# YukunXia/SuperPoint-Stereo-Visual-Odometry

Measured on AMD Instinct MI355X. Metric: stereo frames/sec (1241x376 KITTI), higher is better.
Workload: dtype f32

## Files before the change

### superpoint-stereo-visual-odometry_amd/csrc/conv_first_pre.hip.h

```cpp
#pragma once
#include <hip/hip_runtime.h>
#include <stdint.h>
#include "conv_mfma.hip.h"
#include "post.hip.h"

namespace spvo {

struct FirstPreArgs {
  const uint8_t *src[4];
  uint8_t *out_u8[4];
  size_t stride;
  int row_off, col_off, crop_rows, crop_cols, identity;
  ResizeTab tab;
  float *in_plane;
  size_t in_per_image;
  float *out;
  const float *w, *bias;
  int H, W, hp, wp, out_ctot, out_coff, cout;
};

template <bool RELU>
__global__ __launch_bounds__(256) void conv_first4_pre_kernel(const FirstPreArgs a) {
  constexpr int TW = 256, LW = TW + 4;
  __shared__ __attribute__((aligned(16))) float s[6 * LW];
  const int tid = threadIdx.x, img = blockIdx.z;
  const int x0 = blockIdx.x * TW, y0 = blockIdx.y * 4;
  const uint8_t *src = a.src[img];
  uint8_t *o8 = a.out_u8[img];
  float *ipl = a.in_plane + (size_t)img * a.in_per_image;
  auto stage = [&](const int cx, const int ry0, const int nrows) {
    const int gx = x0 - 1 + cx;
    const bool col_ok = gx >= 0 && gx < a.W;
    const int gxc = col_ok ? gx : 0;
    int xs0 = 0, xs1 = 0, a0 = 0, a1 = 0;
    if (!a.identity) { xs0 = a.tab.xi[gxc]; xs1 = min(xs0 + 1, a.crop_cols - 1); a0 = a.tab.xa0[gxc]; a1 = a.tab.xa1[gxc]; }
    int vv[6];
#pragma unroll
    for (int k = 0; k < 6; ++k) {
      if (k >= nrows) break;
      const int gy = y0 - 1 + ry0 + k;
      const int gyc = min(max(gy, 0), a.H - 1);
      if (a.identity) {
        vv[k] = src[(size_t)(a.row_off + gyc) * a.stride + a.col_off + gxc];
      } else {
        const int ys0 = a.tab.yi[gyc], ys1 = min(ys0 + 1, a.crop_rows - 1);
        const int b0 = a.tab.yb0[gyc], b1 = a.tab.yb1[gyc];
        const uint8_t *r0 = src + (size_t)(a.row_off + ys0) * a.stride + a.col_off;
        const uint8_t *r1 = src + (size_t)(a.row_off + ys1) * a.stride + a.col_off;
        const int h0 = (int)r0[xs0] * a0 + (int)r0[xs1] * a1;
        const int h1 = (int)r1[xs0] * a0 + (int)r1[xs1] * a1;
        const int v = (((b0 * (h0 >> 4)) >> 16) + ((b1 * (h1 >> 4)) >> 16) + 2) >> 2;
        vv[k] = min(max(v, 0), 255);
      }
    }
#pragma unroll
    for (int k = 0; k < 6; ++k) {
      if (k >= nrows) break;
      const int ry = ry0 + k, gy = y0 - 1 + ry;
      const bool ok = col_ok && gy >= 0 && gy < a.H;
      const float f = ok ? mul_rn((float)vv[k], 1.0f / 255.0f) : 0.f;
      if (ok && ry >= 1 && ry <= 4 && cx >= 1 && cx <= TW) {
        if (o8) o8[(size_t)gy * a.W + gx] = (uint8_t)vv[k];
        ipl[(size_t)(gy + PADY) * a.wp + (gx + PADX)] = f;
      }
      s[ry * LW + 3 + cx] = f;
    }
  };
  stage(tid, 0, 6);
  if (tid < 12) stage(TW + (tid & 1), tid >> 1, 1);
  __syncthreads();
  const int l = tid & 63, r = tid >> 6;
  const int x = x0 + 4 * l, y = y0 + r;
  if (x >= a.W || y >= a.H) return;
  float v[3][6];
#pragma unroll
  for (int ky = 0; ky < 3; ++ky) {
    const float *rp = s + (r + ky) * LW + 4 + 4 * l;
    const float4 m = *reinterpret_cast<const float4 *>(rp);
    v[ky][0] = rp[-1]; v[ky][1] = m.x; v[ky][2] = m.y; v[ky][3] = m.z; v[ky][4] = m.w; v[ky][5] = rp[4];
  }
  const size_t plane = (size_t)a.hp * a.wp;
  float *op = a.out + ((size_t)img * a.out_ctot + a.out_coff) * plane + (size_t)(y + PADY) * a.wp + (x + PADX);
  for (int co = 0; co < a.cout; ++co) {
    float sum[4];
#pragma unroll
    for (int i = 0; i < 4; ++i) {
      sum[i] = a.bias[co];
#pragma unroll
      for (int t = 0; t < 9; ++t) sum[i] = fmaf(a.w[co * 9 + t], v[t / 3][i + t % 3], sum[i]);
      if (RELU) sum[i] = fmaxf(sum[i], 0.f);
    }
    *reinterpret_cast<float4 *>(op + (size_t)co * plane) = make_float4(sum[0], sum[1], sum[2], sum[3]);
  }
}

}
```

### superpoint-stereo-visual-odometry_amd/csrc/spvo_core.hip

```cpp
#include "spvo_internal.hip.h"
#include <mutex>

namespace spvo_int {

thread_local std::string g_error;
HostDiag g_diag;

int fail(spvo_ctx *c, int code, const char *fmt, ...) {
  char buf[512];
  va_list ap;
  va_start(ap, fmt);
  vsnprintf(buf, sizeof buf, fmt, ap);
  va_end(ap);
  if (c) c->error = buf;
  g_error = buf;
  return code;
}

int stage_id(spvo_ctx *c, const std::string &name) {
  for (size_t i = 0; i < c->stages.size(); ++i)
    if (c->stages[i].name == name) return (int)i;
  Stage s;
  s.name = name;
  c->stages.push_back(s);
  return (int)c->stages.size() - 1;
}

namespace {
const char *const kTuningNames[] = {"winograd", "wino4", "wino4_item", "wino_narrow", "wino_dynamic", "winograd_min_tiles", "wino4_min_tiles", "merge_siblings", "heads_fused",
                                    "heads_on_net", "heads_split", "match_fused", "fp32_split", "prematch", "spin_wait", "trunk_timing", "solve_timing", "nms_first", "upload_side", "inject_launch_failure", "int8_fused", "pair_always", "preprocess_fused", "heads_keep_raw", "tail_streams", "solve_collect_first", "graphs", "solve_fuse", "solve_keep", "sift_describe_form", "sift_pair_waves_per_cu", "sift_brisk_recheck", "conv_variant"};
constexpr int kTuningCount = sizeof kTuningNames / sizeof kTuningNames[0];
std::mutex g_tuning_mutex;
bool g_tuning_set[kTuningCount] = {};
int g_tuning_value[kTuningCount] = {};
int tuning_index(const char *name) {
  for (int i = 0; name && i < kTuningCount; ++i)
    if (std::strcmp(name, kTuningNames[i]) == 0) return i;
  return -1;
}
}
int tuning(const char *name, int dflt) {
  const int i = tuning_index(name);
  if (i < 0) return dflt;
  std::lock_guard<std::mutex> lock(g_tuning_mutex);
  return g_tuning_set[i] ? g_tuning_value[i] : dflt;
}

bool spin_wait_enabled() { return tuning("spin_wait", 0) != 0; }
hipError_t wait_event(hipEvent_t ev) {
  if (spin_wait_enabled()) {
    for (long spins = 0; spins < 20000000; ++spins) {
      const hipError_t e = hipEventQuery(ev);
      if (e != hipErrorNotReady) return e;
      __builtin_ia32_pause();
    }
  }
  return hipEventSynchronize(ev);
}

hipEvent_t get_event(spvo_ctx *c) {
  if (!c->free_events.empty()) {
    hipEvent_t e = c->free_events.back();
    c->free_events.pop_back();
    return e;
  }
  hipEvent_t e;
  (void)hipEventCreate(&e);
  return e;
}

void resolve_pending(spvo_ctx *c) {
  if (c->pending.empty()) return;
  for (auto &p : c->pending) {
    float ms = 0;
    (void)hipEventSynchronize(p.e1);
    if (hipEventElapsedTime(&ms, p.e0, p.e1) == hipSuccess) {
      c->stages[p.stage].total_ms += ms;
      c->stages[p.stage].calls += 1;
      c->stages[p.stage].flops_sum += p.flops;
      c->stages[p.stage].bytes_sum += p.bytes;
    }
    c->free_events.push_back(p.e0);
    c->free_events.push_back(p.e1);
  }
  c->pending.clear();
}

__thread LaunchRecorder *t_rec = nullptr;

static void seg_drop(GraphEntry &e) {
  if (e.exec) (void)hipGraphExecDestroy(e.exec);
  if (e.graph) (void)hipGraphDestroy(e.graph);
  e = GraphEntry();
}

void set_release_segments(SubmitSet &s) {
  for (GraphEntry *e : {&s.seg_T[0], &s.seg_T[1], &s.seg_H[0], &s.seg_H[1], &s.seg_A, &s.seg_B}) seg_drop(*e);
}
void seg_free_all(spvo_ctx *c) {
  for (SubmitSet &s : c->sets) set_release_segments(s);
}

void seg_abort(spvo_ctx *c) {
  LaunchRecorder &r = c->rec;
  if (t_rec == &r) t_rec = nullptr;
  r.active = false; r.poisoned = false;
  r.rec.clear();
}

bool seg_begin(spvo_ctx *c, GraphEntry *e, hipStream_t stream) {
  LaunchRecorder &r = c->rec;
  if (t_rec == &r) seg_abort(c);
  if (!c->use_graphs || !e || e->never || t_rec) return false;
// ... 412 lines not shown
```

### superpoint-stereo-visual-odometry_amd/csrc/spvo_detect.hip

```cpp
#include "spvo_internal.hip.h"
#include "conv_mfma.hip.h"
#include "post.hip.h"
#include "conv_first_pre.hip.h"

namespace spvo_int {

static void linear_coeffs(int dst, int src, std::vector<int> &idx, std::vector<int> &a0, std::vector<int> &a1) {
  const double scale = (double)src / (double)dst;
  idx.resize(dst); a0.resize(dst); a1.resize(dst);
  for (int d = 0; d < dst; ++d) {
    float f = (float)((d + 0.5) * scale - 0.5);
    int s = (int)std::floor(f);
    f -= (float)s;
    if (s < 0) { s = 0; f = 0.f; }
    if (s >= src - 1) { s = src - 1; f = 0.f; }
    idx[d] = s;
    a0[d] = (int)std::nearbyint((1.f - f) * 2048.f);
    a1[d] = (int)std::nearbyint(f * 2048.f);
  }
}

void resize_tables(int dst_w, int src_w, int dst_h, int src_h, std::vector<int> &out) {
  std::vector<int> xi, xa0, xa1, yi, yb0, yb1;
  linear_coeffs(dst_w, src_w, xi, xa0, xa1);
// ... 14 lines not shown
  }
  g.scale = (float)net_w / (float)g.crop_cols;
  return g;
}

void fix_projection(double P[12], const CropGeom &g, int rows, int cols, int bug_compat) {
  if (bug_compat) {
    float lo;
    if (g.crop_rows != rows) {
      std::memcpy(&lo, (char *)&P[4 + 1], 4);
      lo -= (float)g.row_off;
      std::memcpy((char *)&P[4 + 1], &lo, 4);
    } else if (g.crop_cols != cols) {
      std::memcpy(&lo, (char *)&P[0 + 1], 4);
      lo -= (float)g.col_off;
      std::memcpy((char *)&P[0 + 1], &lo, 4);
    }
  } else {
    if (g.crop_rows != rows) P[4 + 2] -= (double)(float)g.row_off;
    else if (g.crop_cols != cols) P[0 + 2] -= (double)(float)g.col_off;
  }
  for (int k = 0; k < 8; ++k) P[k] *= (double)g.scale;
}

int ensure_tables(spvo_ctx *c, const CropGeom &g) {
  if (c->tab_rows == g.crop_rows && c->tab_cols == g.crop_cols) return SPVO_OK;
  std::vector<int> all;
  resize_tables(c->W, g.crop_cols, c->H, g.crop_rows, all);
  HIP_TRY(c, hipMemcpyAsync(c->d_tab, all.data(), all.size() * sizeof(int), hipMemcpyHostToDevice, c->stream));
  HIP_TRY(c, hipStreamSynchronize(c->stream));
  c->tab_rows = g.crop_rows;
  c->tab_cols = g.crop_cols;
  return SPVO_OK;
}

static ResizeTab resize_tab(const spvo_ctx *c) {
  ResizeTab t;
  t.xi = c->d_tab; t.xa0 = c->d_tab + c->W; t.xa1 = c->d_tab + 2 * c->W;
  t.yi = c->d_tab + 3 * c->W; t.yb0 = t.yi + c->H; t.yb1 = t.yi + 2 * c->H;
  return t;
}

static int ensure_img_staging(spvo_ctx *c, size_t bytes) {
  if (bytes <= c->d_img[1].count()) return SPVO_OK;
  return grow(c, wait_for_nothing(), {plain(c->d_img[0], bytes), plain(c->d_img[1], bytes)});
}

int launch_preprocess(spvo_ctx *c, const uint8_t *d_src0, const uint8_t *d_src1, int count, int rows, int cols, size_t stride, const CropGeom &g, int slot0,
                      uint8_t *resized_dst = nullptr) {
  int rc = ensure_tables(c, g);
  if (rc) return rc;
  ResizeTab tab = resize_tab(c);
  const Tensor &tin = c->tensors[c->t_input];
  const int identity = (g.crop_rows == c->H && g.crop_cols == c->W) ? 1 : 0;
  dim3 grid((c->W + 63) / 64, (c->H + 3) / 4, count);
  hipLaunchKernelGGL(preprocess_kernel, grid, dim3(256), 0, c->stream, d_src0, d_src1, stride, rows, cols, g.row_off, g.col_off, g.crop_rows, g.crop_cols, tab, c->H, c->W,
                     resized_dst ? resized_dst : c->d_resized + (size_t)(slot0 & 1) * c->H * c->W, tin.d + (size_t)slot0 * tin.per_image, tin.per_image, tin.hp, tin.wp, identity);
  HIP_TRY(c, hipGetLastError());
  return SPVO_OK;
}

int launch_first_pre(spvo_ctx *c, PendingDetect *const *mem, int n, hipStream_t stream) {
  const Op &op = c->ops[0];
  const Tensor &ti = c->tensors[op.in], &to = c->tensors[op.out];
  const CropGeom &g = mem[0]->g;
  FirstPreArgs a;
  for (int k = 0; k < 4; ++k) { a.src[k] = nullptr; a.out_u8[k] = nullptr; }
  const size_t hw = (size_t)c->H * c->W;
  for (int m = 0; m < n; ++m)
    for (int i = 0; i < 2; ++i) {
      a.src[2 * m + i] = mem[m]->src[i];
      a.out_u8[2 * m + i] = mem[m]->res_dst ? mem[m]->res_dst + i * hw : (m == n - 1 ? c->d_resized + i * hw : nullptr);
    }
  a.stride = mem[0]->stride;
  a.row_off = g.row_off; a.col_off = g.col_off; a.crop_rows = g.crop_rows; a.crop_cols = g.crop_cols;
  a.identity = (g.crop_rows == c->H && g.crop_cols == c->W) ? 1 : 0;
  a.tab = resize_tab(c);
  a.in_plane = ti.d; a.in_per_image = ti.per_image;
  a.out = ring_ptr(c, to);
  a.w = op.d_w; a.bias = op.d_b;
  a.H = ti.H; a.W = ti.W; a.hp = ti.hp; a.wp = ti.wp; a.out_ctot = to.ch; a.out_coff = op.out_c_off; a.cout = op.cout;
  const int batch = 2 * n;
  ScopedStage st(c, op.stage, op.flops_per_image * batch, 0.0, stream);
  const dim3 grid((ti.W + 255) / 256, (ti.H + 3) / 4, batch);
  if (op.flags & FLAG_RELU) hipLaunchKernelGGL(conv_first4_pre_kernel<true>, grid, dim3(256), 0, stream, a);
  else hipLaunchKernelGGL(conv_first4_pre_kernel<false>, grid, dim3(256), 0, stream, a);
  HIP_TRY(c, hipGetLastError());
  return SPVO_OK;
}

constexpr int NMS_INNER = 4;
constexpr int NMS_GRID = 128;

NmsPair nms_pair(const SubmitSet &s, int *counters) {
  NmsPair p;
  for (int i = 0; i < 2; ++i) {
    p.b[i] = s.nms[i];
    p.b[i].counters = counters + (size_t)i * NMS_COUNTER_INTS;
  }
  return p;
}

int launch_nms_rounds(spvo_ctx *c, int nimg, const NmsPair &np, const SubmitSet &s, int n_launch, int *zero_next, bool redo = false) {
  hipStream_t st = c->post;
  const float *heat = s.d_heat;
  const int collect = redo ? 0 : 1;
  const int n_round = (!redo && n_launch > 1) ? n_launch - 1 : n_launch;
  for (int l = 0; l < n_round; ++l) {
    if (c->cfg.dist_thresh == 4)
      hipLaunchKernelGGL((nms_round_kernel<NMS_INNER, 4>), dim3(NMS_GRID, nimg), dim3(256), 0, st, heat, c->H, c->W, 4, np, l, c->cfg.border_remove, c->surv_cap, collect);
    else
      hipLaunchKernelGGL((nms_round_kernel<NMS_INNER, 0>), dim3(NMS_GRID, nimg), dim3(256), 0, st, heat, c->H, c->W, c->cfg.dist_thresh, np, l, c->cfg.border_remove, c->surv_cap, collect);
  }
  if (n_round < n_launch) {
    if (c->cfg.dist_thresh == 4)
      hipLaunchKernelGGL((nms_finish_kernel<4>), dim3(nimg), dim3(NMS_FIN_THREADS), 0, st, heat, c->H, c->W, 4, np, n_round, c->cfg.border_remove, c->surv_cap);
    else
      hipLaunchKernelGGL((nms_finish_kernel<0>), dim3(nimg), dim3(NMS_FIN_THREADS), 0, st, heat, c->H, c->W, c->cfg.dist_thresh, np, n_round, c->cfg.border_remove, c->surv_cap);
  }
  if (redo) hipLaunchKernelGGL(nms_collect_kernel, dim3(NMS_GRID, nimg), dim3(256), 0, st, heat, c->H, c->W, c->cfg.border_remove, c->surv_cap, np);
  hipLaunchKernelGGL(nms_rank_kernel, dim3(128, nimg), dim3(256), 0, st, c->surv_cap, np);
  hipLaunchKernelGGL(nms_write_kernel, dim3(32, nimg), dim3(256), 0, st, c->H, c->cfg.max_keypoints, c->surv_cap, np, zero_next, s.h_counters);
  HIP_TRY(c, hipGetLastError());
  return SPVO_OK;
}


int nms_settle(spvo_ctx *c, int nimg, const NmsPair &np, const SubmitSet &s, bool *redone) {
  int last = c->nms_first;
  *redone = false;
  const int *hc = s.h_counters;
  for (;;) {
    bool pending = false;
    for (int i = 0; i < nimg; ++i) pending |= hc[i * NMS_COUNTER_INTS + 8 + last - 1] != 0;
    if (!pending) break;
    if (!*redone) c->stages[stage_id(c, "nms_redo")].calls += 1;
    *redone = true;
    last = NMS_MAX_LAUNCH;
    for (int i = 0; i < nimg; ++i)
      HIP_TRY(c, hipMemsetAsync(np.b[i].counters + 1, 0, (NMS_COUNTER_INTS - 1) * sizeof(int), c->post));
    int rc = launch_nms_rounds(c, nimg, np, s, last, nullptr, true);
    if (rc) return rc;
    HIP_TRY(c, hipStreamSynchronize(c->post));
  }
  for (int i = 0; i < nimg; ++i)
    if (hc[i * NMS_COUNTER_INTS + 3]) return fail(c, SPVO_ERR_CAPACITY, "NMS survivor buffer overflow");
  return SPVO_OK;
}

int run_nms(spvo_ctx *c, int nimg) {
  SubmitSet &s = standalone(c);
  const NmsPair np = nms_pair(s, c->d_counters_alone);
  for (int i = 0; i < nimg; ++i) HIP_TRY(c, hipMemsetAsync(np.b[i].counters, 0, NMS_COUNTER_INTS * sizeof(int), c->stream));
  dim3 grid((c->W + 63) / 64, (c->H + 3) / 4, nimg);
  hipLaunchKernelGGL(nms_threshold_kernel, grid, dim3(256), 0, c->stream, s.d_heat, c->H, c->W, c->cfg.conf_thresh, np);
  int rc = launch_nms_rounds(c, nimg, np, s, c->nms_first, nullptr);
  if (rc) return rc;
  HIP_TRY(c, hipStreamSynchronize(c->stream));
  bool redone;
  return nms_settle(c, nimg, np, s, &redone);
}

}

extern "C" {

int spvo_preprocess(spvo_ctx *c, const uint8_t *img, int rows, int cols, size_t stride, double P[12], uint8_t *resized_u8) {
  if (!c || !img || !P || rows <= 0 || cols <= 0 || stride < (size_t)cols) return fail(c, SPVO_ERR_INVALID, "bad argument");
  if (int rc = require_idle(c)) return rc;
// ... 588 lines not shown
```

### superpoint-stereo-visual-odometry_amd/csrc/spvo_internal.hip.h

```cpp
#pragma once
#include <hip/hip_runtime.h>

#include <algorithm>
#include <cmath>
#include <cstdarg>
#include <cstdio>
#include <cstdlib>
#include <cstring>
#include <string>
#include <vector>
#include <deque>
#include <functional>
#include <time.h>

#include "../../include/spvo.h"
#include "spvo_types.hip.h"
#include "engine_file.h"

#pragma GCC visibility push(hidden)
#include "dev_buf.h"
namespace spvo { struct BriskLongPair; struct BriskShortPair; }
using namespace spvo;

#include "launch_segments.hip.h"
// ... 408 lines not shown
    DevBuf<AkazeKp> sup_kp;
    int brk_cap = 0;
    DevBuf<BriskDetKeypoint> brk_rec, brk_crec;
    DevBuf<int> brk_keep, brk_cnt;
  } akaze;
  struct SiftBufs {
    int rows = 0, cols = 0;
    SiftPyr plan{};
    bool gauss_only = false;
    int first = -1;
    DevBuf<SiftKey> given_kp;
    DevBuf<float> given_desc;
    int given_cap = 0;
    int cand_cap = 0;
    DevBuf<uint8_t> img;
    DevBuf<float> pyr, desc;
    DevBuf<int4> cand_pos;
    DevBuf<float4> cand_off;
    DevBuf<int2> kp;
    DevBuf<int> counters;
    std::vector<int4> h_pos;
    std::vector<float4> h_off;
    std::vector<int2> h_kp;
    std::vector<float> h_desc;
    std::vector<spvo_sift_keypoint> h_rec;
    std::vector<int> h_order;
    int ord_cap = 0;
    DevBuf<SiftKey> keys;
    DevBuf<int> sorted, order;
    DevBuf<int> ord_n;
    int slot_cap = 0;
    SiftSlot slots[N_SIFT_SLOTS];
    PairStage pair;
    PinBuf<SiftSrc> h_src;
    PinBuf<float> hm_desc;
    PinBuf<int> h_n;
    PinBuf<int2> h_match;
    int h_match_cap = 0;
    bool match_pending = false;
    int lnk_cap = 0;
    DevBuf<int> lnk_kept, lnk_cnt, lnk_keep;
    int brk_cap = 0;
    DevBuf<BriskDetKeypoint> brk_rec, brk_crec;
    DevBuf<int> brk_keep, brk_cnt;
    PinBuf<SiftSrc> hb_src;
    PinBuf<int> hb_n;
    std::vector<BriskDetKeypoint> hb_rec;
  } sift;
  int ham_cap = 0;
  DevBuf<uint32_t> d_ham_a, d_ham_b;
  DevBuf<int> d_ham_idx;
  DevBuf<float> d_ham_dist;
  DevBuf<unsigned long long> d_ham_vote;
  DevBuf<int2> d_ham_out;
  int bin_pm_norm = SPVO_NORM_HAMMING;
  static constexpr int SOLVE_SLOTS = 3;
  static constexpr int SOLVE_BUFS = 4;
  bool tail_deferred = false;
  int tail_slot = -1;
  alignas(16) char tail_args[320];
  int solve_fuse = 1;
  DevBuf<int> x_counts[SOLVE_BUFS];
  DevBuf<double> x_poses[SOLVE_BUFS];
  DevBuf<ObsDev> x_obs[SOLVE_BUFS];
  struct SolvePending { int n = 0, refinement_degree = 0, slot = 0, frame_count = 0; bool late = false; double rvec[3] = {0, 0, 0}, tvec[3] = {0, 0, 0}; };
  std::deque<SolvePending> solve_q;
  int solve_next_slot = 0;
  int solve_last_slot = -1, solve_last_n = 0;
  hipEvent_t ev_solve[SOLVE_BUFS] = {};
  int solve_cap = 0;
  struct SolveSet {
    DevBuf<char> d_in, d_o;
    DevBuf<double> d_res;
    PinBuf<char> h_in, h_o;
    PinBuf<double> h_res;
  } solve_set[SOLVE_BUFS];
  DevBuf<int> d_ctl;

  bool prof = false;
  int prof_only = -1;
  std::vector<Stage> stages;
  std::vector<Pending> pending;
  bool pre_fused = false;
  bool heads_on_net = false;
  std::vector<hipEvent_t> free_events;
};

namespace spvo_int {

struct HostDiag { double t_last_submit = 0, max_interval = 0, max_tail_wait = 0, max_solve_wait = 0; int match_miss = 0, late = 0, depth_sum = 0;
                  double iv_tail = 0, iv_match = 0, iv_solve = 0; int iv_printed = 0; long launches = 0; };
extern HostDiag g_diag;
inline double diag_now_us() { timespec ts; clock_gettime(CLOCK_MONOTONIC, &ts); return ts.tv_sec * 1e6 + ts.tv_nsec * 1e-3; }

int fail(spvo_ctx *c, int code, const char *fmt, ...);

#define HIP_TRY(c, expr)                                                                     \
  do {                                                                                       \
    hipError_t _e = (expr);                                                                  \
    if (_e != hipSuccess)                                                                    \
      return fail(c, SPVO_ERR_DEVICE, "%s failed: %s (%s:%d)", #expr, hipGetErrorString(_e), \
                  __FILE__, __LINE__);                                                       \
  } while (0)

template <typename T>
int dev_alloc(spvo_ctx *c, T **p, size_t count, bool zero = true) {
  HIP_TRY(c, hipMalloc((void **)p, std::max<size_t>(count, 1) * sizeof(T)));
  if (zero) HIP_TRY(c, hipMemsetAsync(*p, 0, std::max<size_t>(count, 1) * sizeof(T), c->stream));
  return SPVO_OK;
}

template <typename T>
int upload(spvo_ctx *c, T **p, const T *src, size_t count) {
  const int rc = dev_alloc(c, p, count, false);
  if (rc) return rc;
  HIP_TRY(c, hipMemcpy(*p, src, count * sizeof(T), hipMemcpyHostToDevice));
  return SPVO_OK;
}
template <typename T>
int upload(spvo_ctx *c, T **p, const std::vector<T> &v) { return upload(c, p, v.data(), v.size()); }

template <typename T, typename... Rest>
void dev_free(T *&p, Rest *&...rest) {
  if (p) { (void)hipFree(p); p = nullptr; }
  if constexpr (sizeof...(rest) > 0) dev_free(rest...);
}

template <typename T, typename... Rest>
void host_free(T *&p, Rest *&...rest) {
  if (p) { (void)hipHostFree(p); p = nullptr; }
  if constexpr (sizeof...(rest) > 0) host_free(rest...);
}

struct GrowWait { hipStream_t stream = nullptr; };
inline GrowWait wait_for(hipStream_t s) { return GrowWait{s}; }
inline GrowWait wait_for_nothing() { return GrowWait{}; }
template <class T> GrowEntry zeroed(DevBuf<T> &b, size_t count) { return grow_entry<true>(b, count); }
template <class T, class P> GrowEntry plain(Buf<T, P> &b, size_t count) { return grow_entry<false>(b, count); }
inline int grow(spvo_ctx *c, GrowWait w, const std::vector<GrowEntry> &list) {
  if (w.stream) HIP_TRY(c, hipStreamSynchronize(w.stream));
  const GrowResult r = grow_list(list, c->stream);
  if (r.code) return fail(c, SPVO_ERR_DEVICE, "%s failed: %s (%s:%d)", r.call, hipGetErrorString((hipError_t)r.code), __FILE__, __LINE__);
  if (r.cleared) HIP_TRY(c, hipStreamSynchronize(c->stream));
  return SPVO_OK;
}

inline int PairStage::ensure(spvo_ctx *c, size_t px) {
  if (!ev_feat) {
    HIP_TRY(c, hipEventCreateWithFlags(&ev_feat, hipEventDisableTiming));
    HIP_TRY(c, hipEventCreateWithFlags(&ev_match, hipEventDisableTiming));
  }
  if (2 * px > h_img.count()) return grow(c, wait_for(c->stream2), {plain(h_img, 2 * px)});
  return SPVO_OK;
}
inline void PairStage::stage(const uint8_t *img_l, const uint8_t *img_r, int rows, int cols, size_t stride) {
  const uint8_t *imgs[2] = {img_l, img_r};
  const size_t px = (size_t)rows * cols;
  for (int k = 0; k < 2; ++k)
    for (int r = 0; r < rows; ++r) std::memcpy(h_img + k * px + (size_t)r * cols, imgs[k] + (size_t)r * stride, cols);
}
inline void PairStage::release() {
  for (hipEvent_t *e : {&ev_feat, &ev_match}) if (*e) { (void)hipEventDestroy(*e); *e = nullptr; }
}

inline int require_idle(spvo_ctx *c) {
  return c->pendq.empty() ? SPVO_OK : fail(c, SPVO_ERR_STATE, "detector submissions are in flight: complete them with spvo_detect_wait first");
// ... 154 lines not shown
```

### superpoint-stereo-visual-odometry_amd/csrc/spvo_plan.hip

```cpp
#include "spvo_internal.hip.h"
#include "conv_mfma.hip.h"

namespace spvo_int {

void free_plan(spvo_ctx *c) {
  seg_free_all(c);
  for (auto &t : c->tensors) {
    if (t.d) (void)hipFree(t.d);
    for (int r = 1; r < RING; ++r) if (t.dr[r]) (void)hipFree(t.dr[r]);
  }
  for (auto &o : c->ops) dev_free(o.d_w, o.d_b, o.d_bn_scale, o.d_bn_shift, o.d_w16, o.d_w8, o.d_ws3, o.d_wq32, o.d_wsel, o.d_qm, o.d_sched);
  dev_free(c->d_heads_w, c->d_heads_w8, c->d_heads_qm, c->d_heads_b);
  c->heads_fused = false;
  c->heads_kind = c->heads_tiles = c->heads_wgs = 0;
  c->tensors.clear(); c->ops.clear(); c->weights = false; c->fp16 = false; c->int8 = false; c->s3 = false;
}

int choose_variant(const spvo_ctx *c, Op &op, const Tensor &ti, bool split) {
  const int ks = op.ks, H = ti.H, W = ti.W, batch = c->cfg.max_batch, num_cus = c->num_cus, co_tiles = op.co_tiles = (op.cout + CO_TILE - 1) / CO_TILE;
  const bool pool = op.flags & FLAG_POOL;
  int ck = 0;
  struct Cand { int wr, wc, ck; double rate; };
  static const Cand k3_f32[] = {{2, 2, 8, 130.0}, {2, 1, 8, 135.0}, {1, 2, 8, 135.0}, {1, 1, 8, 133.0}};
  static const Cand k3_s3[] = {{2, 2, 8, 108.0}, {2, 1, 8, 100.0}, {1, 2, 8, 97.0}, {1, 1, 8, 97.0}};
// ... 165 lines not shown
    if (op.cin == 1 || tr.ch != op.cout || tr.level != ti.level || tr.nhwc || op.residual == op.out)
      return fail(c, SPVO_ERR_IO, "op %u: bad residual tensor", i);
  }
  if (bn) {
    if (r.bn_off + 4ull * op.cout + 1 > nfl) return fail(c, SPVO_ERR_IO, "op %u: BatchNorm parameters out of range", i);
    const int co_pad = ((op.cout + CO_TILE - 1) / CO_TILE) * CO_TILE;
    const float *q = f.payload + r.bn_off;
    std::vector<float> sc(co_pad, 0.f), sh(co_pad, 0.f);
    for (int o = 0; o < op.cout; ++o) {
      const double k = (double)q[o] / std::sqrt((double)q[3 * op.cout + o] + (double)q[4 * op.cout]);
      sc[o] = (float)k;
      sh[o] = (float)((double)q[op.cout + o] - (double)q[2 * op.cout + o] * k);
    }
    if (c->int8 && to.i8 && !add) {
      const float inv = 1.f / to.scale;
      for (int o = 0; o < op.cout; ++o) { sc[o] = sc[o] * inv; sh[o] = sh[o] * inv; }
    }
    int rc = upload(c, &op.d_bn_scale, sc);
    if (rc || (rc = upload(c, &op.d_bn_shift, sh))) return rc;
  }
  if (op.ks != 1 && op.ks != 3) return fail(c, SPVO_ERR_IO, "op %u: kernel size %d", i, op.ks);
  if (r.w_off + (uint64_t)op.cout * op.cin * taps > nfl || r.b_off + op.cout > nfl) return fail(c, SPVO_ERR_IO, "op %u: weights out of range", i);
  if (op.in_c_off + op.cin > ti.ch || op.out_c_off + op.cout > to.ch) return fail(c, SPVO_ERR_IO, "op %u: channel slice out of range", i);
  const bool pool = op.flags & FLAG_POOL;
  if (to.level != ti.level + (pool ? 1 : 0)) return fail(c, SPVO_ERR_IO, "op %u: level mismatch", i);
  if (pool && ((ti.H | ti.W) & 1)) return fail(c, SPVO_ERR_IO, "op %u: pooling an odd-sized map", i);
  op.flops_per_image = 2.0 * ti.H * ti.W * op.cout * op.cin * taps;
  const float *w = f.payload + r.w_off;
  const float *b = f.payload + r.b_off;
  std::vector<float> wcat, bcat;
  if (!c->s3 && op.ks == 3 && op.cin > 1 && !bn && !add && !pool && (op.cout % CO_TILE) == 0 && i + 1 < f.ops.size() &&
      tuning("merge_siblings", 1)) {
    Op &nx = c->ops[i + 1];
    const EngineOp &rn = f.ops[i + 1];
    if (nx.type == OP_CONV && nx.in == op.in && nx.in_c_off == op.in_c_off && nx.cin == op.cin && nx.ks == op.ks && nx.flags == op.flags &&
        nx.out == op.out && nx.out_c_off == op.out_c_off + op.cout && nx.out_c_off + nx.cout <= to.ch &&
        rn.w_off + (uint64_t)nx.cout * nx.cin * taps <= nfl && rn.b_off + nx.cout <= nfl) {
      wcat.assign(w, w + (size_t)op.cout * op.cin * taps);
      wcat.insert(wcat.end(), f.payload + rn.w_off, f.payload + rn.w_off + (size_t)nx.cout * nx.cin * taps);
      bcat.assign(b, b + op.cout);
      bcat.insert(bcat.end(), f.payload + rn.b_off, f.payload + rn.b_off + nx.cout);
      w = wcat.data();
      b = bcat.data();
      op.cout += nx.cout;
      op.flops_per_image = 2.0 * ti.H * ti.W * op.cout * op.cin * taps;
      nx.merged = true;
    }
  }
  return c->int8 ? prepare_conv_i8(c, i, w, b) : c->fp16 ? prepare_conv_f16(c, i, w, b) : c->s3 ? prepare_conv_s3(c, i, w, b) : prepare_conv_f32(c, i, w, b);
}

int prepare_ops(spvo_ctx *c, const EngineFile &f) {
  for (unsigned i = 0; i < c->ops.size(); ++i) {
    Op &op = c->ops[i];
    const Tensor &ti = c->tensors[op.in], &to = c->tensors[op.out];
    const char *kind = op.type == OP_DWCONV ? "dwconv" : op.type == OP_CONV ? "conv" : op.type == OP_MAXPOOL ? "pool" : op.type == OP_L2NORM ? "l2norm" : nullptr;
    if (!kind) return fail(c, SPVO_ERR_IO, "op %u: unknown type %d", i, op.type);
    char name[64];
    std::snprintf(name, sizeof name, "%s:%u", kind, i);
    op.stage = stage_id(c, name);
    int rc = SPVO_OK;
    if (op.type == OP_DWCONV) rc = prepare_dwconv(c, f, i);
    else if (op.type == OP_CONV && !op.merged) rc = prepare_conv(c, f, i);
    else if (op.type == OP_MAXPOOL && (to.level != ti.level + 1 || to.ch != ti.ch)) rc = fail(c, SPVO_ERR_IO, "op %u: bad pool", i);
    else if (op.type == OP_L2NORM && (ti.ch != 256 || to.ch != 256 || ti.level != 3)) rc = fail(c, SPVO_ERR_IO, "op %u: descriptor tail must be 256 channels at 1/8", i);
    if (rc) return rc;
  }
  return SPVO_OK;
}

int fuse_tail(spvo_ctx *c, const EngineFile &f) {
  if (c->s3 || c->head_start + 3 != c->ops.size() || !tuning("heads_fused", 1)) return SPVO_OK;
  const EngineOp &rp = f.ops[c->head_start], &rd = f.ops[c->head_start + 1];
  return c->int8 ? fuse_tail_i8(c, f.payload, rp, rd) : fuse_tail_f32(c, f.payload, rp, rd);
}

void place(spvo_ctx *c) {
  Op *best = nullptr;
  for (auto &o : c->ops) if (o.type == OP_CONV && (!best || o.flops_per_image > best->flops_per_image)) best = &o;
  if (best) best->dominant = true;
  const Op &o0 = c->ops[0];
  c->pre_fused = !c->fp16 && !c->int8 && !c->s3 && c->head_start >= 1 && o0.type == OP_CONV && o0.cin == 1 && o0.ks == 3 && o0.in == c->t_input && !o0.d_bn_scale &&
                 !(o0.flags & (FLAG_POOL | FLAG_ADD)) && !c->tensors[o0.out].nhwc && (c->W % 8) == 0 && tuning("preprocess_fused", 1) != 0;
  if (c->pendq.empty()) c->tail_streams = tuning("tail_streams", 0) == 2 ? 2 : 1;
  double all = 0, big = 0;
  for (const auto &o : c->ops) if (o.type == OP_CONV) { all += o.flops_per_image; if (o.wino4) big += o.flops_per_image; }
  c->heads_on_net = big > 0.8 * all;
  c->use_graphs = tuning("graphs", 1) == 2 || ((c->fp16 || c->int8) && tuning("graphs", 1) != 0);
}

int check_bindings(spvo_ctx *c, const char *path) {
  const Tensor &td = c->tensors[c->t_det];
  const Tensor &ts = c->tensors[c->t_desc];
  if (td.ch != 65 || td.level != 3 || td.nhwc || !ts.nhwc || c->tensors[c->t_input].ch != 1 || c->tensors[c->t_input].level != 0)
    return fail(c, SPVO_ERR_IO, "%s: unexpected output tensors", path);
  return SPVO_OK;
}

}
}

extern "C" int spvo_load_weights(spvo_ctx *c, const char *path) {
  if (!c || !path) return fail(c, SPVO_ERR_INVALID, "null argument");
  HIP_TRY(c, hipSetDevice(c->cfg.device));
  std::vector<unsigned char> bytes;
  int rc = read_engine_file(c, path, bytes);
  if (rc) return rc;
  const EngineFile f = parse_engine_file(bytes.data(), bytes.size(), c->H, path);
  if (f.status) return fail(c, f.status, "%s", f.error.c_str());
  if (!c->pendq.empty()) return fail(c, SPVO_ERR_STATE, "detector submissions are in flight");
  free_plan(c);
  build_tensors_and_ops(c, f);
  if ((rc = assign_storage(c, f, path))) return rc;
  find_heads(c);
  if ((rc = alloc_activations(c))) return rc;
  if ((rc = prepare_ops(c, f))) return rc;
  if ((rc = fuse_tail(c, f))) return rc;
  if (c->int8 && tuning("int8_fused", 1)) plan_int8_fusion(c);
  place(c);
  if ((rc = check_bindings(c, path))) return rc;
  HIP_TRY(c, hipStreamSynchronize(c->stream));
  c->weights = true;
  return SPVO_OK;
}
```

Measured before the change: 1628.

## Stage first-layer conv weights in LDS and align output stores to 128B

The fused preprocess plus first-conv kernel now loads bias and 3x3 weights per output channel into shared memory, padded to a 12-float pitch, and reads them as float4 instead of issuing scalar global loads inside the channel loop. A second form shifts the tile origin so that each thread's float4 output stores line up with 128-byte boundaries. Each wave handles two aligned windows with alternating channels, which needs extra left halo columns and possibly an extra block column. New tuning flags select the form, with fallbacks when the alignment or shared-memory budget conditions fail.

```diff
diff --git a/superpoint-stereo-visual-odometry_amd/csrc/conv_first_pre.hip.h b/superpoint-stereo-visual-odometry_amd/csrc/conv_first_pre.hip.h
--- a/superpoint-stereo-visual-odometry_amd/csrc/conv_first_pre.hip.h
+++ b/superpoint-stereo-visual-odometry_amd/csrc/conv_first_pre.hip.h
@@ -19,17 +19,36 @@
   int H, W, hp, wp, out_ctot, out_coff, cout;
 };
 
-template <bool RELU>
+constexpr int FIRST_PRE_WPITCH = 12, FIRST_PRE_LDS_BUDGET = 160 * 1024 / 8;
+constexpr int first_pre_left(int form) { return form == 2 ? 29 : 1; }
+constexpr int first_pre_lw(int form) { return 256 + first_pre_left(form) + 3; }
+constexpr int first_pre_tile_floats(int form) { return 6 * first_pre_lw(form) + 4; }
+inline size_t first_pre_lds_bytes(int form, int cout) { return ((size_t)first_pre_tile_floats(form) + (form ? (size_t)cout * FIRST_PRE_WPITCH : 0)) * sizeof(float); }
+inline int first_pre_blocks_x(int form, int W) { return (W + first_pre_left(form) - 1 + 255) / 256; }
+
+template <bool RELU, int FORM = 2, int UNROLL = 2>
 __global__ __launch_bounds__(256) void conv_first4_pre_kernel(const FirstPreArgs a) {
-  constexpr int TW = 256, LW = TW + 4;
-  __shared__ __attribute__((aligned(16))) float s[6 * LW];
+  constexpr bool LDSW = FORM != 0, ALIGN = FORM == 2;
+  constexpr int TW = 256, XL = first_pre_left(FORM), NX = XL + 1, LW = first_pre_lw(FORM);
+  extern __shared__ __attribute__((aligned(16))) float s[];
+  float *const sw = s + first_pre_tile_floats(FORM);
   const int tid = threadIdx.x, img = blockIdx.z;
+  const int wn = LDSW ? a.cout * FIRST_PRE_WPITCH : 0;
+  auto wfetch = [&](const int j) {
+    const int co = j / FIRST_PRE_WPITCH, k = j - co * FIRST_PRE_WPITCH;
+    return j >= wn || k > 9 ? 0.f : k == 0 ? a.bias[co] : a.w[co * 9 + k - 1];
+  };
+  float w0[3] = {0.f, 0.f, 0.f};
+  if (LDSW) {
+#pragma unroll
+    for (int k = 0; k < 3; ++k) w0[k] = wfetch(tid + 256 * k);
+  }
   const int x0 = blockIdx.x * TW, y0 = blockIdx.y * 4;
   const uint8_t *src = a.src[img];
   uint8_t *o8 = a.out_u8[img];
   float *ipl = a.in_plane + (size_t)img * a.in_per_image;
   auto stage = [&](const int cx, const int ry0, const int nrows) {
-    const int gx = x0 - 1 + cx;
+    const int gx = x0 - XL + cx;
     const bool col_ok = gx >= 0 && gx < a.W;
     const int gxc = col_ok ? gx : 0;
     int xs0 = 0, xs1 = 0, a0 = 0, a1 = 0;
@@ -59,7 +78,7 @@
       const int ry = ry0 + k, gy = y0 - 1 + ry;
       const bool ok = col_ok && gy >= 0 && gy < a.H;
       const float f = ok ? mul_rn((float)vv[k], 1.0f / 255.0f) : 0.f;
-      if (ok && ry >= 1 && ry <= 4 && cx >= 1 && cx <= TW) {
+      if (ok && ry >= 1 && ry <= 4 && cx >= XL && cx < XL + TW) {
         if (o8) o8[(size_t)gy * a.W + gx] = (uint8_t)vv[k];
         ipl[(size_t)(gy + PADY) * a.wp + (gx + PADX)] = f;
       }
@@ -67,30 +86,77 @@
     }
   };
   stage(tid, 0, 6);
-  if (tid < 12) stage(TW + (tid & 1), tid >> 1, 1);
+  if (tid < 6 * NX) stage(TW + tid % NX, tid / NX, 1);
+  if (LDSW) {
+#pragma unroll
+    for (int k = 0; k < 3; ++k)
+      if (tid + 256 * k < wn) sw[tid + 256 * k] = w0[k];
+    for (int j = tid + 768; j < wn; j += 256) sw[j] = wfetch(j);
+  }
   __syncthreads();
   const int l = tid & 63, r = tid >> 6;
-  const int x = x0 + 4 * l, y = y0 + r;
-  if (x >= a.W || y >= a.H) return;
-  float v[3][6];
+  const int y = y0 + r;
+  if (y >= a.H) return;
+  const size_t plane = (size_t)a.hp * a.wp;
+  float *const orow = a.out + ((size_t)img * a.out_ctot + a.out_coff) * plane + (size_t)(y + PADY) * a.wp + PADX;
+  struct Window { float v[3][6]; bool ok; float *op; };
+  auto window = [&](const int xs) {
+    Window wd;
+    const int x = xs + 4 * l;
+    wd.ok = x >= 0 && x < a.W;
 #pragma unroll
-  for (int ky = 0; ky < 3; ++ky) {
-    const float *rp = s + (r + ky) * LW + 4 + 4 * l;
-    const float4 m = *reinterpret_cast<const float4 *>(rp);
-    v[ky][0] = rp[-1]; v[ky][1] = m.x; v[ky][2] = m.y; v[ky][3] = m.z; v[ky][4] = m.w; v[ky][5] = rp[4];
-  }
-  const size_t plane = (size_t)a.hp * a.wp;
-  float *op = a.out + ((size_t)img * a.out_ctot + a.out_coff) * plane + (size_t)(y + PADY) * a.wp + (x + PADX);
-  for (int co = 0; co < a.cout; ++co) {
+    for (int ky = 0; ky < 3; ++ky) {
+      const float *rp = s + (r + ky) * LW + 3 + XL + (x - x0);
+      const float4 m = *reinterpret_cast<const float4 *>(rp);
+      wd.v[ky][0] = rp[-1]; wd.v[ky][1] = m.x; wd.v[ky][2] = m.y; wd.v[ky][3] = m.z; wd.v[ky][4] = m.w; wd.v[ky][5] = rp[4];
+    }
+    wd.op = orow + x;
+    return wd;
+  };
+  auto channel = [&](const Window &wd, const float b, const float (&wt)[9], const int co) {
     float sum[4];
 #pragma unroll
     for (int i = 0; i < 4; ++i) {
-      sum[i] = a.bias[co];
+      sum[i] = b;
 #pragma unroll
-      for (int t = 0; t < 9; ++t) sum[i] = fmaf(a.w[co * 9 + t], v[t / 3][i + t % 3], sum[i]);
+      for (int t = 0; t < 9; ++t) sum[i] = fmaf(wt[t], wd.v[t / 3][i + t % 3], sum[i]);
       if (RELU) sum[i] = fmaxf(sum[i], 0.f);
     }
-    *reinterpret_cast<float4 *>(op + (size_t)co * plane) = make_float4(sum[0], sum[1], sum[2], sum[3]);
+    *reinterpret_cast<float4 *>(wd.op + (size_t)co * plane) = make_float4(sum[0], sum[1], sum[2], sum[3]);
+  };
+  struct Weights { float4 q0, q1, q2; };
+  auto weights = [&](const int co) {
+    const float4 *const q = reinterpret_cast<const float4 *>(sw) + co * 3;
+    return Weights{q[0], q[1], q[2]};
+  };
+  auto channel_lds = [&](const Window &wd, const Weights &k, const int co) {
+    const float wt[9] = {k.q0.y, k.q0.z, k.q0.w, k.q1.x, k.q1.y, k.q1.z, k.q1.w, k.q2.x, k.q2.y};
+    channel(wd, k.q0.x, wt, co);
+  };
+  if (!ALIGN) {
+    const Window wd = window(x0);
+    if (!wd.ok) return;
+    if (!LDSW) {
+      for (int co = 0; co < a.cout; ++co) {
+        float wt[9];
+#pragma unroll
+        for (int t = 0; t < 9; ++t) wt[t] = a.w[co * 9 + t];
+        channel(wd, a.bias[co], wt, co);
+      }
+    } else {
+#pragma unroll UNROLL
+      for (int co = 0; co < a.cout; ++co) channel_lds(wd, weights(co), co);
+    }
+    return;
+  }
+  const int sa = (int)((reinterpret_cast<uintptr_t>(orow + x0) >> 2) & 31), sb = (int)((sa + plane) & 31);
+  const Window wa = window(x0 - sa), wb = window(x0 - sb);
+  if (!wa.ok && !wb.ok) return;
+  for (int co = 0; co < a.cout; co += 2) {
+    const bool odd = co + 1 < a.cout;
+    const Weights ka = weights(co), kb = weights(odd ? co + 1 : co);
+    if (wa.ok) channel_lds(wa, ka, co);
+    if (wb.ok && odd) channel_lds(wb, kb, co + 1);
   }
 }
 
diff --git a/superpoint-stereo-visual-odometry_amd/csrc/spvo_core.hip b/superpoint-stereo-visual-odometry_amd/csrc/spvo_core.hip
--- a/superpoint-stereo-visual-odometry_amd/csrc/spvo_core.hip
+++ b/superpoint-stereo-visual-odometry_amd/csrc/spvo_core.hip
@@ -28,7 +28,7 @@
 
 namespace {
 const char *const kTuningNames[] = {"winograd", "wino4", "wino4_item", "wino_narrow", "wino_dynamic", "winograd_min_tiles", "wino4_min_tiles", "merge_siblings", "heads_fused",
-                                    "heads_on_net", "heads_split", "match_fused", "fp32_split", "prematch", "spin_wait", "trunk_timing", "solve_timing", "nms_first", "upload_side", "inject_launch_failure", "int8_fused", "pair_always", "preprocess_fused", "heads_keep_raw", "tail_streams", "solve_collect_first", "graphs", "solve_fuse", "solve_keep", "sift_describe_form", "sift_pair_waves_per_cu", "sift_brisk_recheck", "conv_variant"};
+                                    "heads_on_net", "heads_split", "match_fused", "fp32_split", "prematch", "spin_wait", "trunk_timing", "solve_timing", "nms_first", "upload_side", "inject_launch_failure", "int8_fused", "pair_always", "preprocess_fused", "heads_keep_raw", "tail_streams", "solve_collect_first", "graphs", "solve_fuse", "solve_keep", "sift_describe_form", "sift_pair_waves_per_cu", "sift_brisk_recheck", "conv_variant", "first_layer_lds", "first_layer_align"};
 constexpr int kTuningCount = sizeof kTuningNames / sizeof kTuningNames[0];
 std::mutex g_tuning_mutex;
 bool g_tuning_set[kTuningCount] = {};
diff --git a/superpoint-stereo-visual-odometry_amd/csrc/spvo_detect.hip b/superpoint-stereo-visual-odometry_amd/csrc/spvo_detect.hip
--- a/superpoint-stereo-visual-odometry_amd/csrc/spvo_detect.hip
+++ b/superpoint-stereo-visual-odometry_amd/csrc/spvo_detect.hip
@@ -120,9 +120,22 @@
   a.H = ti.H; a.W = ti.W; a.hp = ti.hp; a.wp = ti.wp; a.out_ctot = to.ch; a.out_coff = op.out_c_off; a.cout = op.cout;
   const int batch = 2 * n;
   ScopedStage st(c, op.stage, op.flops_per_image * batch, 0.0, stream);
-  const dim3 grid((ti.W + 255) / 256, (ti.H + 3) / 4, batch);
-  if (op.flags & FLAG_RELU) hipLaunchKernelGGL(conv_first4_pre_kernel<true>, grid, dim3(256), 0, stream, a);
-  else hipLaunchKernelGGL(conv_first4_pre_kernel<false>, grid, dim3(256), 0, stream, a);
+  int form = !c->first_lds ? 0 : !c->first_align ? 1 : 2;
+  if (form == 2 && (((2 * (size_t)a.hp * a.wp) & 31) || (reinterpret_cast<uintptr_t>(a.out) & 15))) form = 1;
+  if (first_pre_lds_bytes(form, op.cout) > (size_t)FIRST_PRE_LDS_BUDGET) form = 0;
+  const dim3 grid(first_pre_blocks_x(form, ti.W), (ti.H + 3) / 4, batch);
+  const size_t lds = first_pre_lds_bytes(form, op.cout);
+  const bool relu = (op.flags & FLAG_RELU) != 0;
+  if (form == 2) {
+    if (relu) hipLaunchKernelGGL((conv_first4_pre_kernel<true, 2>), grid, dim3(256), lds, stream, a);
+    else hipLaunchKernelGGL((conv_first4_pre_kernel<false, 2>), grid, dim3(256), lds, stream, a);
+  } else if (form == 1) {
+    if (relu) hipLaunchKernelGGL((conv_first4_pre_kernel<true, 1>), grid, dim3(256), lds, stream, a);
+    else hipLaunchKernelGGL((conv_first4_pre_kernel<false, 1>), grid, dim3(256), lds, stream, a);
+  } else {
+    if (relu) hipLaunchKernelGGL((conv_first4_pre_kernel<true, 0>), grid, dim3(256), lds, stream, a);
+    else hipLaunchKernelGGL((conv_first4_pre_kernel<false, 0>), grid, dim3(256), lds, stream, a);
+  }
   HIP_TRY(c, hipGetLastError());
   return SPVO_OK;
 }
diff --git a/superpoint-stereo-visual-odometry_amd/csrc/spvo_internal.hip.h b/superpoint-stereo-visual-odometry_amd/csrc/spvo_internal.hip.h
--- a/superpoint-stereo-visual-odometry_amd/csrc/spvo_internal.hip.h
+++ b/superpoint-stereo-visual-odometry_amd/csrc/spvo_internal.hip.h
@@ -514,6 +514,8 @@
   std::vector<Stage> stages;
   std::vector<Pending> pending;
   bool pre_fused = false;
+  bool first_lds = true;
+  bool first_align = true;
   bool heads_on_net = false;
   std::vector<hipEvent_t> free_events;
 };
diff --git a/superpoint-stereo-visual-odometry_amd/csrc/spvo_plan.hip b/superpoint-stereo-visual-odometry_amd/csrc/spvo_plan.hip
--- a/superpoint-stereo-visual-odometry_amd/csrc/spvo_plan.hip
+++ b/superpoint-stereo-visual-odometry_amd/csrc/spvo_plan.hip
@@ -271,6 +271,8 @@
   const Op &o0 = c->ops[0];
   c->pre_fused = !c->fp16 && !c->int8 && !c->s3 && c->head_start >= 1 && o0.type == OP_CONV && o0.cin == 1 && o0.ks == 3 && o0.in == c->t_input && !o0.d_bn_scale &&
                  !(o0.flags & (FLAG_POOL | FLAG_ADD)) && !c->tensors[o0.out].nhwc && (c->W % 8) == 0 && tuning("preprocess_fused", 1) != 0;
+  c->first_lds = tuning("first_layer_lds", 1) != 0;
+  c->first_align = tuning("first_layer_align", 1) != 0;
   if (c->pendq.empty()) c->tail_streams = tuning("tail_streams", 0) == 2 ? 2 : 1;
   double all = 0, big = 0;
   for (const auto &o : c->ops) if (o.type == OP_CONV) { all += o.flops_per_image; if (o.wino4) big += o.flops_per_image; }
```

After: 1635, median of 6. About the same (+0.4%).
